# tkwong/parameter_server

Hardware: AMD Instinct MI355X
Metric: device-resident KV Add+Get GB/s (grad+param bytes) at 1/2/4/8 GPU (higher is better)
Workload: dtype f32; 1 GPU; cfg 2 dense: 1e8-key float shard, 64 x 1000000 contiguous-key windows at 1M-aligned bases pushed, then windows the push did not touch pulled (zero push/pull overlap), per step; assign (last-write-wins) mode, grouped launches, 16 window sets rotated over the steps; key_space=100000000, batch_keys=1000000, window_sets=16, push_pull_overlap_keys=0, parallelism=range-sharded x1 (no collective)

## Files before the change

### parameter_server_amd/csrc/pskv_internal.h

```cpp
#pragma once
#include <hip/hip_runtime.h>
#include <stddef.h>
#include <stdint.h>

#include "pskv_plan.h"

namespace pskv {

constexpr int kBlock = 256;
constexpr int kGatherVec = 4;
constexpr int kSortedUnroll = 2;
inline int stream_chunk(int unroll) { return kBlock * 4 * unroll; }
constexpr int kSortedChunk = kBlock * 4 * kSortedUnroll;
constexpr int kGeneralChunk = 2048;
constexpr int kGeneralSlots = 4096;
constexpr int kRbBinBlockDefault = 1024;
constexpr uint32_t kRbMaxSc = 1024;
constexpr int kInlineMax = 256;
constexpr int kInlineGetMax = 512;
constexpr int kInlineMaxChunks = 16;
constexpr unsigned long long kEmpty64 = ~0ull;
constexpr uint32_t kEmpty32 = 0xFFFFFFFFu;

constexpr uint32_t kErrOverflowFull = 1u;
// ... 77 lines not shown
};
static_assert(sizeof(OvfMbox) == 128, "device and host words on separate 64-byte lines");
struct OvfCtl {
  OvfTab t;
  uint32_t stat[2];
  OvfMbox* mbox;
};
struct Ovf {
  OvfCtl* c;
};

hipError_t launch_gather(int vb, bool vec, int unroll, bool nt, const GroupArgs& ga,
                         uint32_t nwg, const DenseView& d, const Ovf& o, hipStream_t st);
hipError_t launch_assign_sorted(int vb, bool vec, const uint32_t* keys, const void* vals,
                                uint64_t n, const DenseView& d, uint32_t* flag, uint32_t epoch,
                                hipStream_t st);
hipError_t launch_assign_group(int vb, bool vec, int unroll, bool nt, bool ntp, bool early,
                               const GroupArgs& ga,
                               const DenseView& d, uint32_t tile_shift, uint64_t ntiles,
                               uint32_t grid, uint32_t* flag, uint32_t epoch, hipStream_t st);
hipError_t launch_general_mark(int dtype, int mode, const GroupArgs& ga, uint32_t nwg,
                               const DenseView& d, uint32_t* oor, unsigned long long* owner,
                               const uint32_t* cond, uint32_t epoch, hipStream_t st);
hipError_t launch_general_commit(int vb, const GroupArgs& ga, uint32_t nwg, const DenseView& d,
                                 const unsigned long long* owner,
                                 const uint32_t* cond, uint32_t epoch, hipStream_t st);
hipError_t launch_ovf_rehash(int vb, const Ovf& o, uint64_t from_cap, const OvfTab& to, hipStream_t st);
hipError_t launch_replay(int dtype, int mode, const GroupArgs& ga, const DenseView& d, const Ovf& o,
                         const uint32_t* cond, uint32_t epoch, hipStream_t st, bool oor_only = false);
constexpr uint32_t kK1rTableWords = 4100;
hipError_t launch_gather_replay(int vb, bool vec, int unroll, bool nt, const GroupArgs& ga, uint32_t nwg,
                                const DenseView& d, const Ovf& o, const ReplayGroup& rg,
                                const uint32_t* cond, uint32_t epoch, uint32_t* tab, hipStream_t st);
hipError_t launch_rb_add(int dtype, int mode, const GroupArgs& ga, uint32_t nsc,
                         const DenseView& d, const Ovf& o, const RbMap& bm,
                         int apply_log2, int bin_block, uint16_t* loff, void* tmp,
                         hipStream_t st);
uint32_t rb_superchunk(int vb, int bin_block);
constexpr size_t kRbTmpPad = 16;
hipError_t launch_inline_add(int dtype, int mode, const InlineAdd& a, const DenseView& d,
                             const Ovf& o, hipStream_t st);
hipError_t launch_inline_get(int vb, const InlineGet& a, const DenseView& d, const Ovf& o,
                             void* out, unsigned int* done, unsigned int seq, hipStream_t st);
hipError_t launch_serve(int dtype, int mode, SrvRing* ring, const DenseView& d, const Ovf& o,
                        void* reply, uint32_t start_seq, unsigned long long idle_ticks,
                        uint32_t gen, hipStream_t st);
size_t rb_entry_bytes(int vb);
hipError_t launch_dense_check(const GroupArgs& ga, uint32_t nchunks, const DenseView& d,
                              uint32_t* flag, uint32_t epoch, hipStream_t st);
hipError_t launch_acc_dense(int dtype, const GroupArgs& ga, uint32_t grid, const DenseView& d,
                            const uint32_t* flag, uint32_t epoch, hipStream_t st);


struct RowShape {
  uint32_t units;
  uint32_t unit_bytes;
  uint32_t lanes;
  uint32_t lshift;
};
RowShape row_shape(uint32_t width, int vb, bool unit16);
hipError_t launch_row_gather(int vb, bool nt, const GroupArgs& ga, uint32_t nwg, const DenseView& d,
                             const RowShape& rs, hipStream_t st);
hipError_t launch_row_commit(int vb, const GroupArgs& ga, uint32_t nwg, const DenseView& d,
                             const unsigned long long* owner, const Ovf& o, uint32_t epoch,
                             const RowShape& rs, hipStream_t st);
hipError_t launch_row_accumulate(int dtype, const GroupArgs& ga, uint32_t nwg, const DenseView& d,
// ... 4 lines not shown
```

### parameter_server_amd/csrc/pskv_kernels.hip

```cpp
#include <type_traits>

#include "pskv_internal.h"

namespace pskv {
namespace {


__device__ __forceinline__ uint32_t fmix32(uint32_t h) {
  h ^= h >> 16;
  h *= 0x85ebca6bu;
  h ^= h >> 13;
  h *= 0xc2b2ae35u;
  h ^= h >> 16;
  return h;
}

typedef unsigned int u32x4 __attribute__((ext_vector_type(4)));

template <bool NT>
__device__ __forceinline__ u32x4 ld16(const void* p) {
  if (NT) return __builtin_nontemporal_load(reinterpret_cast<const u32x4*>(p));
  return *reinterpret_cast<const u32x4*>(p);
}
template <bool NT>
// ... 292 lines not shown
  if (run && (off0 & 3u) == 0u) {
    Vec4<VT>::template load<NTP>(reinterpret_cast<const VT*>(d.param) + off0, v);
  } else if (sizeof(VT) == 4 && run) {
    uint32_t t[4];
    ld16a4<NTP>(reinterpret_cast<const uint32_t*>(d.param) + off0, t);
#pragma unroll
    for (int e = 0; e < 4; ++e) v[e] = (VT)t[e];
  } else {
#pragma unroll
    for (int e = 0; e < 4; ++e) v[e] = load_one<VT, FRESH>(d, o, k[e]);
  }
}

template <bool FRESH = false>
__device__ __forceinline__ void gather2(const DenseView& d, const Ovf& o, const uint32_t (&k)[2],
                                        unsigned long long (&v)[2]) {
  using T = unsigned long long;
  const uint32_t off0 = k[0] - d.key_begin;
  const bool run = (k[1] == k[0] + 1u) & ((uint64_t)off0 + 1u < d.range);
  if (run && (off0 & 1u) == 0u) {
    Vec2x8::load(reinterpret_cast<const T*>(d.param) + off0, v);
  } else if (run) {
    uint32_t t[4];
    ld16a4<false>(reinterpret_cast<const uint32_t*>(reinterpret_cast<const T*>(d.param) + off0), t);
    v[0] = (T)t[0] | ((T)t[1] << 32);
    v[1] = (T)t[2] | ((T)t[3] << 32);
  } else {
    v[0] = load_one<T, FRESH>(d, o, k[0]);
    v[1] = load_one<T, FRESH>(d, o, k[1]);
  }
}

struct GoAlways {
  __device__ bool operator()() const { return true; }
};
template <typename VT, bool VEC, int U, bool NT, typename Go = GoAlways, bool FRESH = false>
__device__ __forceinline__ void gather_chunk(const GroupArgs& ga, const DenseView& d, const Ovf& o,
                                             uint32_t wg, Go go = Go()) {
  constexpr int CH = kBlock * 4 * U;
  const int j = batch_of(ga, wg);
  const uint32_t* __restrict__ keys = ga.b[j].keys;
  VT* __restrict__ out = reinterpret_cast<VT*>(const_cast<void*>(ga.b[j].vals));
  const uint64_t n = ga.b[j].n;
  const uint64_t base = (uint64_t)(wg - ga.wg_prefix[j]) * CH;
  const int tid = threadIdx.x;
  if constexpr (sizeof(VT) == 8) {
    if (VEC && base + CH <= n) {
      constexpr int UU = 2 * U;
      uint32_t k[UU][2];
#pragma unroll
      for (int u = 0; u < UU; ++u) ld8_keys<NT>(keys + base + (uint64_t)(u * kBlock + tid) * 2, k[u]);
      if (!go()) return;
      VT v[UU][2];
#pragma unroll
      for (int u = 0; u < UU; ++u) gather2<FRESH>(d, o, k[u], v[u]);
#pragma unroll
      for (int u = 0; u < UU; ++u) Vec2x8::store<NT>(out + base + (uint64_t)(u * kBlock + tid) * 2, v[u]);
      return;
    }
  }
  STEP_STAMP(1, 0);
  if (VEC && base + CH <= n) {
    uint32_t k[U][4];
#pragma unroll
    for (int u = 0; u < U; ++u)
      Vec4<uint32_t>::load<NT>(keys + base + (uint64_t)(u * kBlock + tid) * 4, k[u]);
    if (!go()) return;
#ifdef PSKV_STEP_STAMPS
    ready(k[0]);
    STEP_STAMP(1, 1);
#endif
    VT v[U][4];
#pragma unroll
    for (int u = 0; u < U; ++u) gather4<VT, false, FRESH>(d, o, k[u], v[u]);
#pragma unroll
    for (int u = 0; u < U; ++u)
      Vec4<VT>::template store<NT>(out + base + (uint64_t)(u * kBlock + tid) * 4, v[u]);
    STEP_STAMP(1, 2);
  } else {
    if (!go()) return;
    const uint64_t end = n < base + CH ? n : base + CH;
    for (uint64_t i0 = base + tid; i0 < end; i0 += 8ull * kBlock) {
      uint32_t kk[8];
      VT vv[8];
#pragma unroll
      for (int q = 0; q < 8; ++q) {
        const uint64_t i = i0 + (uint64_t)q * kBlock;
        kk[q] = i < end ? keys[i] : 0u;
      }
#pragma unroll
      for (int q = 0; q < 8; ++q)
        vv[q] = i0 + (uint64_t)q * kBlock < end ? load_one<VT, FRESH>(d, o, kk[q]) : VT(0);
#pragma unroll
      for (int q = 0; q < 8; ++q) {
        const uint64_t i = i0 + (uint64_t)q * kBlock;
        if (i < end) out[i] = vv[q];
      }
    }
  }
}

template <typename VT, bool VEC, int U, bool NT>
__global__ __launch_bounds__(kBlock) void k_gather(GroupArgs ga, DenseView d, Ovf o) {
  gather_chunk<VT, VEC, U, NT>(ga, d, o, blockIdx.x);
}


template <typename VT>
__device__ __forceinline__ bool scalar_elem(const uint32_t* __restrict__ keys,
                                            const VT* __restrict__ vals, uint64_t n, uint64_t i,
                                            const DenseView& d, uint64_t lo, uint64_t hi) {
  const uint32_t k = keys[i];
  const bool hn = i + 1 < n;
  const uint32_t nk = hn ? keys[i + 1] : 0u;
// ... 1368 lines not shown
          } else {
            const long long sl = ovf_insert(o, ot, key[q]);
            if (sl >= 0) reinterpret_cast<VT*>(ot.vals)[sl] = v[q];
          }
        } else {
          if (!(own >> q & 1u)) continue;
          VT* p = nullptr;
          if ((uint64_t)off < d.range) {
            p = reinterpret_cast<VT*>(d.param) + off;
          } else {
            const long long sl = ovf_insert(o, ot, key[q]);
            if (sl >= 0) p = reinterpret_cast<VT*>(ot.vals) + sl;
          }
          if (p) *p = add_wrap<VT>(*p, hsum[slot[q]]);
        }
      }
      __syncthreads();
    }
  }
}

template <typename VT, int MODE, bool OOR_ONLY>
__global__ __launch_bounds__(kReplayBlock) void k_replay(GroupArgs ga, DenseView d, Ovf o,
                                                         const uint32_t* cond, uint32_t epoch) {
  constexpr int SLOTS = replay_slots<kReplayBlock>();
  __shared__ uint32_t hk[SLOTS];
  __shared__ uint32_t hidx[MODE == 0 ? SLOTS + 1 : 1];
  __shared__ VT hsum[MODE == 1 ? SLOTS + 1 : 1];
  __shared__ uint32_t sent;
  if (*cond != epoch) return;
  replay_group<VT, MODE, kReplayBlock, GroupArgs, OOR_ONLY>(ga, d, o, hk, hidx, hsum, &sent);
}

template <typename VT, bool VEC, int U, bool NT>
__global__ __launch_bounds__(kBlock) void k_gather_r(GroupArgs ga, DenseView d, Ovf o, ReplayGroup rg,
                                                     const uint32_t* cond, uint32_t epoch, uint32_t* tab) {
  const uint32_t tag = *cond;
  bool tagged = false;
  gather_chunk<VT, VEC, U, NT>(ga, d, o, blockIdx.x, [&]() {
    tagged = tag == epoch;
    return !tagged;
  });
  if (tagged && blockIdx.x == 0) {
    constexpr int SLOTS = replay_slots<kBlock>();
    static_assert(2 * SLOTS + 2 <= (int)kK1rTableWords, "K1r's replay table fits its scratch");
    replay_group<VT, 0, kBlock>(rg, d, o, tab, tab + SLOTS, static_cast<VT*>(nullptr), tab + 2 * SLOTS + 1);
    for (uint32_t w = 0; w < gridDim.x; ++w) gather_chunk<VT, VEC, U, NT, GoAlways, true>(ga, d, o, w);
  }
}


template <int U>
__global__ __launch_bounds__(kBlock) void k_dense_check(GroupArgs ga, DenseView d, uint32_t* flag,
                                                        uint32_t epoch) {
  constexpr int CH = kBlock * 4 * U;
  const uint32_t wg = blockIdx.x;
  const int j = batch_of(ga, wg);
  const uint32_t* __restrict__ keys = ga.b[j].keys;
  const uint64_t n = ga.b[j].n;
  const uint64_t base = (uint64_t)(wg - ga.wg_prefix[j]) * CH;
  const int tid = threadIdx.x;
  const uint32_t first = keys[0];
  const uint64_t off = (uint32_t)(first - d.key_begin);
  bool bad = off >= d.range || off + n > d.range;
  if (base + CH <= n && (reinterpret_cast<uintptr_t>(keys) & 15u) == 0) {
    uint32_t k[U][4];
#pragma unroll
    for (int u = 0; u < U; ++u)
      Vec4<uint32_t>::load<true>(keys + base + (uint64_t)(u * kBlock + tid) * 4, k[u]);
#pragma unroll
    for (int u = 0; u < U; ++u) {
      const uint32_t k0 = first + (uint32_t)(base + (uint64_t)(u * kBlock + tid) * 4);
      bad |= (k[u][0] != k0) | (k[u][1] != k0 + 1u) | (k[u][2] != k0 + 2u) | (k[u][3] != k0 + 3u);
    }
  } else {
    const uint64_t end = n < base + CH ? n : base + CH;
    for (uint64_t i = base + tid; i < end; i += kBlock) bad |= keys[i] != first + (uint32_t)i;
  }
  if (__any(bad) && (tid & 63) == 0) *flag = epoch;
}
// ... 408 lines not shown
                                   const Ovf& o, const ReplayGroup& rg, const uint32_t* cond, uint32_t epoch,
                                   uint32_t* tab, hipStream_t st) {
  if (unroll == 8) {
    if (nt)
      k_gather_r<VT, VEC, 8, true><<<nwg, kBlock, 0, st>>>(ga, d, o, rg, cond, epoch, tab);
    else
      k_gather_r<VT, VEC, 8, false><<<nwg, kBlock, 0, st>>>(ga, d, o, rg, cond, epoch, tab);
  } else {
    if (nt)
      k_gather_r<VT, VEC, 4, true><<<nwg, kBlock, 0, st>>>(ga, d, o, rg, cond, epoch, tab);
    else
      k_gather_r<VT, VEC, 4, false><<<nwg, kBlock, 0, st>>>(ga, d, o, rg, cond, epoch, tab);
  }
}

hipError_t launch_gather_replay(int vb, bool vec, int unroll, bool nt, const GroupArgs& ga, uint32_t nwg,
                                const DenseView& d, const Ovf& o, const ReplayGroup& rg,
                                const uint32_t* cond, uint32_t epoch, uint32_t* tab, hipStream_t st) {
  if (nwg == 0) return hipErrorInvalidValue;
  if (vb == 4) {
    if (vec)
      gather_replay_dispatch<uint32_t, true>(unroll, nt, nwg, ga, d, o, rg, cond, epoch, tab, st);
    else
      gather_replay_dispatch<uint32_t, false>(unroll, nt, nwg, ga, d, o, rg, cond, epoch, tab, st);
  } else {
    if (vec)
      gather_replay_dispatch<unsigned long long, true>(unroll, nt, nwg, ga, d, o, rg, cond, epoch, tab, st);
    else
      gather_replay_dispatch<unsigned long long, false>(unroll, nt, nwg, ga, d, o, rg, cond, epoch, tab, st);
  }
  return hipGetLastError();
}

hipError_t launch_assign_sorted(int vb, bool vec, const uint32_t* keys, const void* vals,
                                uint64_t n, const DenseView& d, uint32_t* flag, uint32_t epoch,
                                hipStream_t st) {
  if (n == 0) return hipSuccess;
  const uint32_t nwg = (uint32_t)((n + kSortedChunk - 1) / kSortedChunk);
  if (vb == 4) {
    auto v = reinterpret_cast<const uint32_t*>(vals);
    if (vec)
      k_assign_sorted<uint32_t, true><<<nwg, kBlock, 0, st>>>(keys, v, n, d, flag, epoch);
    else
      k_assign_sorted<uint32_t, false><<<nwg, kBlock, 0, st>>>(keys, v, n, d, flag, epoch);
  } else {
    auto v = reinterpret_cast<const unsigned long long*>(vals);
    if (vec)
      k_assign_sorted<unsigned long long, true><<<nwg, kBlock, 0, st>>>(keys, v, n, d, flag, epoch);
    else
      k_assign_sorted<unsigned long long, false><<<nwg, kBlock, 0, st>>>(keys, v, n, d, flag, epoch);
  }
  return hipGetLastError();
}

#ifndef PSKV_K2G_LDS_CAP
#define PSKV_K2G_LDS_CAP (48u << 10)
#endif
constexpr uint32_t kK2gLdsCap = PSKV_K2G_LDS_CAP;

template <typename VT, bool VEC, bool NTP>
static void group_dispatch2(int unroll, bool nt, bool early, uint32_t grid, const GroupArgs& ga,
                            const DenseView& d, uint32_t shift, uint64_t ntiles, uint32_t* flag,
                            uint32_t epoch, hipStream_t st) {
  const uint32_t cap = sizeof(VT) == 4 && VEC && unroll == 8 ? kK2gLdsCap : 0u;
  if constexpr (sizeof(VT) == 4 && VEC) {
    if (early && unroll == 8 && nt) {
// ... 255 lines not shown
```

### parameter_server_amd/csrc/pskv_plan.h

```cpp
#pragma once
#include <stddef.h>
#include <stdint.h>

#include <algorithm>
#include <cstring>
#include <utility>
#include <vector>

#include "pskv.h"

namespace pskv {

constexpr int kMaxBatches = 64;
constexpr int kRbMaxBuckets = 2064;
constexpr uint64_t kMaxGroupElems = 1ull << 32;

constexpr size_t kPieceBytes = 1 << 20;
constexpr size_t kCheckPieceBytes = 256 << 10;
constexpr size_t kWindowBytes = 8 << 20;

namespace {

static inline size_t round16(size_t x) { return (x + 15) & ~size_t(15); }

// ... 17 lines not shown
                                             uint64_t max_elems = kMaxGroupElems) {
  std::vector<Span> out;
  size_t b = 0;
  while (b < v.size()) {
    size_t e = b;
    uint64_t el = 0;
    while (e < v.size() && e - b < max_batches && el + v[e].n < max_elems) {
      el += v[e].n;
      ++e;
    }
    out.emplace_back(b, e);
    b = e;
  }
  return out;
}

static inline std::vector<Span> batch_windows(const std::vector<pskv_batch>& v, size_t min_key_bytes = kWindowBytes,
                                              size_t max_batches = kMaxBatches,
                                              uint64_t max_elems = kMaxGroupElems) {
  std::vector<Span> wins;
  for (size_t i = 0; i < v.size();) {
    size_t j = i, kb = 0;
    uint64_t el = 0;
    while (j < v.size() &&
           (j == i || (kb < min_key_bytes && j - i < max_batches && el + v[j].n < max_elems))) {
      kb += v[j].n * 4;
      el += v[j].n;
      ++j;
    }
    wins.emplace_back(i, j);
    i = j;
  }
  return wins;
}

enum class StageOrder {
  kInterleaved,
  kKeysFirst,
};
struct StageSlot {
  size_t keys, vals;
};
struct StageLayout {
  std::vector<StageSlot> at;
  size_t key_bytes = 0;
  size_t total = 0;
  std::vector<pskv_batch> views(const std::vector<pskv_batch>& v, char* base) const {
    std::vector<pskv_batch> out(v.size());
    for (size_t i = 0; i < v.size(); ++i)
      out[i] = pskv_batch{reinterpret_cast<const uint32_t*>(base + at[i].keys), base + at[i].vals, v[i].n};
    return out;
  }
};

static inline size_t staged_bytes(const std::vector<pskv_batch>& v, size_t vb) {
  size_t bytes = 0;
  for (const auto& b : v) bytes += round16(b.n * 4) + round16(b.n * vb);
  return bytes;
}

static inline StageLayout stage_layout(const std::vector<pskv_batch>& v, size_t vb, StageOrder order) {
  StageLayout l;
  l.at.resize(v.size());
  for (const auto& b : v) l.key_bytes += round16(b.n * 4);
  size_t ko = 0, vo = order == StageOrder::kKeysFirst ? l.key_bytes : 0;
  for (size_t i = 0; i < v.size(); ++i) {
// ... 146 lines not shown
```

### parameter_server_amd/csrc/pskv_shard.cpp

```cpp
#include <hip/hip_runtime.h>

#include <algorithm>
#include <cctype>
#include <cerrno>
#include <atomic>
#include <chrono>
#include <condition_variable>
#include <cstdio>
#include <cstdlib>
#include <cstring>
#include <functional>
#include <mutex>
#include <string>
#include <thread>
#include <vector>

#include "pskv.h"
#include "pskv_frames.h"
#include "pskv_internal.h"
#include "pskv_plan.h"
#include "pskv_queues.h"

using namespace pskv;

// ... 197 lines not shown
  uint32_t tune_rb_wbits = 0;
  uint32_t tune_rb_nbd = 0;
  bool tune_inline = true;
  int tune_inline_add_chunks = 1;
  int tune_inline_get_chunks = 2;
  void* ireply = nullptr;
  bool tune_ispin = true;
  unsigned int ireply_seq = 0;
  int tune_rb_apply_log2 = 0;
  int tune_rb_bin_block = kRbBinBlockDefault;
  bool tune_serve = false;
  uint32_t tune_serve_idle_us = 20000;
  SrvRing* srv = nullptr;
  uint32_t srv_gen = 0;
  hipStream_t srv_stream = nullptr;
  hipEvent_t srv_dep = nullptr;
  bool srv_running = false;
  uint32_t srv_posted = 0;
  unsigned long long srv_idle_ticks = 0;
  bool counted = false;
  bool add_chunks_set = false;
  int wall_khz = 0;
  uint32_t tune_sync_timeout_ms = 120000;
  int last_kernel = -1;
  uint64_t launches = 0;
  hipEvent_t sync_ev = nullptr;
  uint32_t* stat_host = nullptr;
  int tune_fold_replay = 1;
  bool defer_replay = false;
  bool pend_replay = false;
  ReplayGroup pend_rg{};
  uint32_t pend_epoch = 0;
  uint64_t pend_elems = 0;

  DenseView dview() const { return DenseView{dense, key_begin, range}; }
};

namespace {

constexpr uint64_t kGetSmallKeys = 24ull << 20;
int gather_unroll(const pskv_shard* s, uint64_t elems) {
  if (s->tune_get_unroll) return s->tune_get_unroll;
  if (s->tune_unroll == 4) return 4;
  return elems < kGetSmallKeys ? 4 : 8;
}

int use_device(pskv_shard* s) {
  PSKV_HIP(hipSetDevice(s->device));
  return PSKV_OK;
}

hipEvent_t take_event(pskv_shard* s) {
  if (!s->event_pool.empty()) {
    hipEvent_t e = s->event_pool.back();
    s->event_pool.pop_back();
    return e;
  }
  hipEvent_t e = nullptr;
  if (hipEventCreateWithFlags(&e, hipEventDisableSystemFence) != hipSuccess) return nullptr;
  return e;
}

struct LaunchTimer {
  pskv_shard* s;
  int kernel;
  uint64_t elems;
// ... 1237 lines not shown
  if (s->width > 1) return rows_get(s, in, flags);
  std::vector<pskv_batch> v;
  for (auto& b : in) {
    if (b.n == 0) continue;
    if (!b.keys || !b.vals) return fail(PSKV_EINVAL, "pskv_get: null keys/out with n > 0");
    push_pieces(v, b, (size_t)s->vb);
  }
  s->n_get++;
  if (v.empty()) return PSKV_OK;
  int rc = use_device(s);
  if (rc) return rc;
  const bool device = (flags & PSKV_DEVICE) != 0;
  if (!device && s->tune_inline) {
    uint64_t total = 0;
    for (const auto& b : v) total += b.n;
    if (total <= (uint64_t)kInlineGetMax * s->tune_inline_get_chunks) return inline_get(s, v, total);
  }
  rc = srv_stop(s);
  if (rc) return rc;
  if (device) return gather_all(s, v, all_aligned16(v), true);
  const size_t bytes = staged_bytes(v, (size_t)s->vb);
  std::vector<pskv_batch> views;
  if (bytes <= s->tune_frame_zc_max_bytes &&
      (((flags & PSKV_HOST_FRAME) && frame_views(v, (size_t)s->vb, &views)) ||
       pinned_views(v, (size_t)s->vb, &views)))
    return zero_copy_get_views(s, views);
  bool pinned = true;
  for (const auto& b : v) pinned = pinned && is_pinned(b.keys) && is_pinned(b.vals);
  if (!pinned && s->tune_zc_max_bytes && bytes <= s->tune_zc_max_bytes) return zero_copy_get(s, v);
  if (!pinned && s->tune_pageable_dma) pinned = bytes >= s->tune_dma_min_bytes_get;
  return pinned ? pinned_get(s, v) : staged_get(s, v);
}

int add_get_impl(pskv_shard* s, const std::vector<pskv_batch>& adds, const std::vector<pskv_batch>& gets,
                 int flags) {
  if (s->width > 1) {
    const int rc = rows_add(s, adds, flags);
    return rc ? rc : rows_get(s, gets, flags);
  }
  s->defer_replay = s->tune_fold_replay && (flags & PSKV_DEVICE) && s->mode == PSKV_ASSIGN && s->vb == 4;
  int rc = add_impl(s, adds, flags);
  s->defer_replay = false;
  if (!rc) rc = get_impl(s, gets, flags & ~PSKV_SORTED_HINT);
  const int rf = flush_replay(s);
  return rc ? rc : rf;
}

struct Option {
  const char* name;
  int64_t lo, hi;
  int64_t (*get)(const pskv_shard*);
  void (*set)(pskv_shard*, int64_t);
};

#define PSKV_OPT(NAME, LO, HI, FIELD, T)                                           \
  Option {                                                                         \
    NAME, LO, HI, [](const pskv_shard* s) -> int64_t { return (int64_t)s->FIELD; }, \
        [](pskv_shard* s, int64_t v) { s->FIELD = (T)v; }                          \
  }

const Option kOptions[] = {
    PSKV_OPT("GENERAL", 0, 2, general_path, int),
    PSKV_OPT("UNROLL", 4, 8, tune_unroll, int),
    PSKV_OPT("GET_UNROLL", 0, 8, tune_get_unroll, int),
    PSKV_OPT("FOLD_REPLAY", 0, 1, tune_fold_replay, int),
    PSKV_OPT("NT", 0, 1, tune_nt, bool),
    PSKV_OPT("NTP", 0, 1, tune_ntp, bool),
    PSKV_OPT("EARLY", 0, 2, tune_early, int),
    PSKV_OPT("PAGEABLE_DMA", 0, 1, tune_pageable_dma, bool),
    PSKV_OPT("DMA_MIN_BYTES", 0, INT64_MAX, tune_dma_min_bytes, size_t),
    PSKV_OPT("DMA_MIN_BYTES_GET", 0, INT64_MAX, tune_dma_min_bytes_get, size_t),
    PSKV_OPT("DMA_MIN_BYTES_PINNED", 0, INT64_MAX, tune_dma_min_bytes_pinned, size_t),
    PSKV_OPT("ZC_MAX_BYTES", 0, INT64_MAX, tune_zc_max_bytes, size_t),
    PSKV_OPT("FRAME_ZC_MAX_BYTES", 0, INT64_MAX, tune_frame_zc_max_bytes, size_t),
    PSKV_OPT("INLINE", 0, 1, tune_inline, bool),
    PSKV_OPT("INLINE_ADD_CHUNKS", 1, kInlineMaxChunks, tune_inline_add_chunks, int),
    PSKV_OPT("INLINE_GET_CHUNKS", 1, kInlineMaxChunks, tune_inline_get_chunks, int),
    PSKV_OPT("ISPIN", 0, 1, tune_ispin, bool),
    PSKV_OPT("SERVE", 0, 1, tune_serve, bool),
    PSKV_OPT("SERVE_IDLE_US", 1, 10000000, tune_serve_idle_us, uint32_t),
    PSKV_OPT("TILE_SHIFT", 0, 20, tune_tile_shift, uint32_t),
    PSKV_OPT("TILE_GRID", 1, 65536, tune_tile_grid, uint32_t),
    PSKV_OPT("RB_WBITS", 0, 31, tune_rb_wbits, uint32_t),
    PSKV_OPT("RB_NBD", 0, kRbMaxBuckets - 1, tune_rb_nbd, uint32_t),
    PSKV_OPT("RB_TB", 0, 11, tune_rb_tb, uint32_t),
    PSKV_OPT("RB_APPLY_LOG2", 0, 14, tune_rb_apply_log2, int),
    PSKV_OPT("RB_BIN_BLOCK", 512, 1024, tune_rb_bin_block, int),
    PSKV_OPT("SYNC_TIMEOUT_MS", 0, 0x7FFFFFFF, tune_sync_timeout_ms, uint32_t),
};
#undef PSKV_OPT

const Option* find_option(const char* name) {
  for (const auto& o : kOptions)
    if (std::strcmp(o.name, name) == 0) return &o;
  return nullptr;
}

int set_option(pskv_shard* s, const Option& o, int64_t v) {
  if (v < o.lo || v > o.hi) return fail(PSKV_EINVAL, std::string("option ") + o.name + ": value out of range");
  if (std::strcmp(o.name, "UNROLL") == 0 && v != 4 && v != 8) return fail(PSKV_EINVAL, "option UNROLL: 4 or 8");
  if (std::strcmp(o.name, "GET_UNROLL") == 0 && v != 0 && v != 4 && v != 8)
    return fail(PSKV_EINVAL, "option GET_UNROLL: 0, 4 or 8");
  if (std::strcmp(o.name, "TILE_SHIFT") == 0 && v != 0 && v < 10) return fail(PSKV_EINVAL, "option TILE_SHIFT: 0 or 10..20");
  if (std::strcmp(o.name, "RB_APPLY_LOG2") == 0 && v != 0 && v != 13 && v != 14)
    return fail(PSKV_EINVAL, "option RB_APPLY_LOG2: 0, 13 or 14");
  if (std::strcmp(o.name, "RB_BIN_BLOCK") == 0 && v != 512 && v != 1024)
    return fail(PSKV_EINVAL, "option RB_BIN_BLOCK: 512 or 1024");
  o.set(s, v);
  if (std::strcmp(o.name, "SYNC_TIMEOUT_MS") == 0) refresh_grow_wait(s);
  if (std::strcmp(o.name, "INLINE_ADD_CHUNKS") == 0) s->add_chunks_set = true;
  if (std::strcmp(o.name, "SERVE") == 0 && !s->add_chunks_set) s->tune_inline_add_chunks = v ? 2 : 1;
  return PSKV_OK;
}

int apply_env_options(pskv_shard* s) {
  static std::mutex warn_mu;
  static std::vector<std::string> warned;
  static const char* const kRetired[] = {"RB_INSERT", "GET_DEDUP", "GET_NTP", "FUSE"};
  for (const char* name : kRetired) {
    const std::string var = std::string("PSKV_") + name;
    const char* e = std::getenv(var.c_str());
// ... 160 lines not shown
  if (s->out_stream) drain(s->out_stream, "D2H output stream (destroy)");
  if (s->own_stream) drain(s->own_stream, "shard stream (destroy)");
  if (s->stream && s->stream != s->own_stream) drain(s->stream, "caller stream (destroy)");
  if (!stuck.empty()) {
    std::fprintf(stderr, "pskv: shard destroy: %s; its device memory and streams are not freed\n", stuck.c_str());
    return fail(PSKV_ESTATE, "pskv_shard_destroy: " + stuck);
  }
  GrowService::get().remove(s);
  if (s->counted) g_queues.add_shard(s->device, -1);
  if (s->out_stream) g_queues.add_stream(s->device, -1);
  if (s->srv) (void)hipHostFree(s->srv);
  if (s->srv_stream) (void)hipStreamDestroy(s->srv_stream);
  if (s->srv_dep) (void)hipEventDestroy(s->srv_dep);
  if (s->out_stream) (void)hipStreamDestroy(s->out_stream);
  for (auto e : s->out_events) (void)hipEventDestroy(e);
  for (auto& t : s->pending) {
    (void)hipEventDestroy(t.a);
    (void)hipEventDestroy(t.b);
  }
  for (auto e : s->event_pool) (void)hipEventDestroy(e);
  if (s->sync_ev) (void)hipEventDestroy(s->sync_ev);
  if (s->dense) (void)hipFree(s->dense);
  if (s->owner) (void)hipFree(s->owner);
  if (s->flag) (void)hipFree(s->flag);
  for (const auto& t : s->tables) {
    (void)hipFree(t.keys);
    (void)hipFree(t.vals);
  }
  if (s->ovf.c) (void)hipFree(s->ovf.c);
  if (s->mbox) (void)hipHostFree(s->mbox);
  if (s->dstage) (void)hipFree(s->dstage);
  if (s->rb_loff) (void)hipFree(s->rb_loff);
  if (s->rb_ent) (void)hipFree(s->rb_ent);
  if (s->hstage) (void)hipHostFree(s->hstage);
  if (s->ireply) (void)hipHostFree(s->ireply);
  if (s->stat_host) (void)hipHostFree(s->stat_host);
  if (s->hstage_free) (void)hipEventDestroy(s->hstage_free);
  if (s->h2d_done) (void)hipEventDestroy(s->h2d_done);
  for (auto e : s->win_events) (void)hipEventDestroy(e);
  if (s->own_stream) (void)hipStreamDestroy(s->own_stream);
  delete s;
  return PSKV_OK;
}

static bool bad_flags(int flags) {
  return (flags & ~(PSKV_DEVICE | PSKV_SORTED_HINT | PSKV_HOST_FRAME)) != 0 ||
         ((flags & PSKV_DEVICE) && (flags & PSKV_HOST_FRAME));
}

int pskv_add(pskv_shard* s, const uint32_t* keys, const void* vals, uint64_t n, int flags) {
  if (!s) return fail(PSKV_EINVAL, "pskv_add: null shard");
  if (bad_flags(flags)) return fail(PSKV_EINVAL, "pskv_add: unknown flags");
  pskv_batch b{keys, const_cast<void*>(vals), n};
  return add_impl(s, std::vector<pskv_batch>{b}, flags);
}

int pskv_get(pskv_shard* s, const uint32_t* keys, uint64_t n, void* out, int flags) {
  if (!s) return fail(PSKV_EINVAL, "pskv_get: null shard");
  if (bad_flags(flags)) return fail(PSKV_EINVAL, "pskv_get: unknown flags");
  pskv_batch b{keys, out, n};
  return get_impl(s, std::vector<pskv_batch>{b}, flags);
}

int pskv_add_grouped(pskv_shard* s, const pskv_batch* batches, uint64_t nb, int flags) {
  if (!s) return fail(PSKV_EINVAL, "pskv_add_grouped: null shard");
  if (nb && !batches) return fail(PSKV_EINVAL, "pskv_add_grouped: null batches");
// ... 226 lines not shown
```

Measured before the change: 6432 GB/s.

## Fuse last push group and first pull group into one concurrent step kernel

Adds a fused step kernel that runs the final assign-add group's workgroups and the first gather group's workgroups in one launch. Gather workgroups check their key range against the push windows with wave ballots and defer any chunk that overlaps a push to a tail kernel, which also handles the replay fallback. A host-side rule reads a device-written report and stops fusing for a while when more than half of the chunks were deferred. The aim is to remove the serialization and launch gap between push and pull so read and write bandwidth overlap. The cost is extra overlap-check work, a tail launch, and added complexity.

New measurement: 6429 GB/s (median of 3 runs). No clear change (-0.0%).

```diff
diff --git a/parameter_server_amd/csrc/pskv_internal.h b/parameter_server_amd/csrc/pskv_internal.h
--- a/parameter_server_amd/csrc/pskv_internal.h
+++ b/parameter_server_amd/csrc/pskv_internal.h
@@ -133,6 +133,20 @@
 hipError_t launch_gather_replay(int vb, bool vec, int unroll, bool nt, const GroupArgs& ga, uint32_t nwg,
                                 const DenseView& d, const Ovf& o, const ReplayGroup& rg,
                                 const uint32_t* cond, uint32_t epoch, uint32_t* tab, hipStream_t st);
+struct FuseCtl {
+  uint32_t* defer;
+  uint32_t* total;
+  unsigned long long* report;
+};
+constexpr int kFuseUnroll = 4;
+static_assert(2 * sizeof(GroupArgs) + 160 <= 4096 && sizeof(GroupArgs) + sizeof(ReplayGroup) + 160 <= 4096,
+              "K10's and K1t's groups plus their other arguments fit the 4 KiB kernarg segment");
+hipError_t launch_step_fused(bool early, const GroupArgs& ga, uint32_t nadd, const GroupArgs& gg, uint32_t nget,
+                             const DenseView& d, const Ovf& o, uint32_t tile_shift, uint64_t ntiles,
+                             uint32_t* flag, uint32_t epoch, const FuseCtl& fc, hipStream_t st);
+hipError_t launch_gather_tail(const GroupArgs& gg, uint32_t nget, uint32_t grid, const DenseView& d, const Ovf& o,
+                              const ReplayGroup& rg, const uint32_t* cond, uint32_t epoch, uint32_t* tab,
+                              const FuseCtl& fc, hipStream_t st);
 hipError_t launch_rb_add(int dtype, int mode, const GroupArgs& ga, uint32_t nsc,
                          const DenseView& d, const Ovf& o, const RbMap& bm,
                          int apply_log2, int bin_block, uint16_t* loff, void* tmp,
diff --git a/parameter_server_amd/csrc/pskv_kernels.hip b/parameter_server_amd/csrc/pskv_kernels.hip
--- a/parameter_server_amd/csrc/pskv_kernels.hip
+++ b/parameter_server_amd/csrc/pskv_kernels.hip
@@ -348,7 +348,11 @@
 }
 
 struct GoAlways {
-  __device__ bool operator()() const { return true; }
+  template <typename K>
+  __device__ bool whole(const K&) const {
+    return true;
+  }
+  __device__ bool part(const uint32_t*, uint64_t, uint64_t) const { return true; }
 };
 template <typename VT, bool VEC, int U, bool NT, typename Go = GoAlways, bool FRESH = false>
 __device__ __forceinline__ void gather_chunk(const GroupArgs& ga, const DenseView& d, const Ovf& o,
@@ -366,7 +370,7 @@
       uint32_t k[UU][2];
 #pragma unroll
       for (int u = 0; u < UU; ++u) ld8_keys<NT>(keys + base + (uint64_t)(u * kBlock + tid) * 2, k[u]);
-      if (!go()) return;
+      if (!go.whole(k)) return;
       VT v[UU][2];
 #pragma unroll
       for (int u = 0; u < UU; ++u) gather2<FRESH>(d, o, k[u], v[u]);
@@ -381,7 +385,7 @@
 #pragma unroll
     for (int u = 0; u < U; ++u)
       Vec4<uint32_t>::load<NT>(keys + base + (uint64_t)(u * kBlock + tid) * 4, k[u]);
-    if (!go()) return;
+    if (!go.whole(k)) return;
 #ifdef PSKV_STEP_STAMPS
     ready(k[0]);
     STEP_STAMP(1, 1);
@@ -394,8 +398,8 @@
       Vec4<VT>::template store<NT>(out + base + (uint64_t)(u * kBlock + tid) * 4, v[u]);
     STEP_STAMP(1, 2);
   } else {
-    if (!go()) return;
     const uint64_t end = n < base + CH ? n : base + CH;
+    if (!go.part(keys, base, end)) return;
     for (uint64_t i0 = base + tid; i0 < end; i0 += 8ull * kBlock) {
       uint32_t kk[8];
       VT vv[8];
@@ -1830,20 +1834,230 @@
   replay_group<VT, MODE, kReplayBlock, GroupArgs, OOR_ONLY>(ga, d, o, hk, hidx, hsum, &sent);
 }
 
+struct GoUntagged {
+  uint32_t tag, epoch;
+  template <typename K>
+  __device__ bool whole(const K&) const {
+    return tag != epoch;
+  }
+  __device__ bool part(const uint32_t*, uint64_t, uint64_t) const { return tag != epoch; }
+};
 template <typename VT, bool VEC, int U, bool NT>
 __global__ __launch_bounds__(kBlock) void k_gather_r(GroupArgs ga, DenseView d, Ovf o, ReplayGroup rg,
                                                      const uint32_t* cond, uint32_t epoch, uint32_t* tab) {
   const uint32_t tag = *cond;
-  bool tagged = false;
-  gather_chunk<VT, VEC, U, NT>(ga, d, o, blockIdx.x, [&]() {
-    tagged = tag == epoch;
-    return !tagged;
-  });
-  if (tagged && blockIdx.x == 0) {
+  gather_chunk<VT, VEC, U, NT>(ga, d, o, blockIdx.x, GoUntagged{tag, epoch});
+  if (tag == epoch && blockIdx.x == 0) {
     constexpr int SLOTS = replay_slots<kBlock>();
     static_assert(2 * SLOTS + 2 <= (int)kK1rTableWords, "K1r's replay table fits its scratch");
     replay_group<VT, 0, kBlock>(rg, d, o, tab, tab + SLOTS, static_cast<VT*>(nullptr), tab + 2 * SLOTS + 1);
     for (uint32_t w = 0; w < gridDim.x; ++w) gather_chunk<VT, VEC, U, NT, GoAlways, true>(ga, d, o, w);
+  }
+}
+
+struct GoDisjoint {
+  const GroupArgs& push;
+  uint32_t epoch;
+  uint32_t* word;
+  uint32_t* total;
+  template <typename Hit>
+  __device__ __forceinline__ bool test(uint32_t lo, uint32_t hi, Hit hit) const {
+    const int lane = threadIdx.x & 63;
+    uint32_t pf = 0, pl = 0;
+    const bool pv = lane < push.nb && push.b[lane].n > 0;
+    if (pv) {
+      pf = push.b[lane].keys[0];
+      pl = push.b[lane].keys[push.b[lane].n - 1];
+    }
+#pragma unroll
+    for (int w = 32; w >= 1; w >>= 1) {
+      lo = min(lo, (uint32_t)__shfl_xor((int)lo, w, 64));
+      hi = max(hi, (uint32_t)__shfl_xor((int)hi, w, 64));
+    }
+    unsigned long long m = __ballot(pv && pf <= hi && pl >= lo);
+    bool h = false;
+    while (m) {
+      const int q = __ffsll((long long)m) - 1;
+      m &= m - 1;
+      h |= hit((uint32_t)__shfl((int)pf, q, 64), (uint32_t)__shfl((int)pl, q, 64));
+    }
+    if (__ballot(h) == 0) return true;
+    if (lane == 0 && atomicExch(word, epoch) != epoch) atomicAdd(total, 1u);
+    return false;
+  }
+  template <int UU>
+  __device__ __forceinline__ bool whole(const uint32_t (&k)[UU][4]) const {
+    uint32_t lo = k[0][0], hi = k[0][0];
+#pragma unroll
+    for (int u = 0; u < UU; ++u)
+#pragma unroll
+      for (int e = 0; e < 4; ++e) {
+        lo = min(lo, k[u][e]);
+        hi = max(hi, k[u][e]);
+      }
+    return test(lo, hi, [&](uint32_t f, uint32_t l) {
+      bool h = false;
+#pragma unroll
+      for (int u = 0; u < UU; ++u)
+#pragma unroll
+        for (int e = 0; e < 4; ++e) h |= (k[u][e] >= f) & (k[u][e] <= l);
+      return h;
+    });
+  }
+  __device__ __forceinline__ bool part(const uint32_t* __restrict__ keys, uint64_t base, uint64_t end) const {
+    uint32_t lo = kEmpty32, hi = 0u;
+    for (uint64_t i = base + threadIdx.x; i < end; i += kBlock) {
+      lo = min(lo, keys[i]);
+      hi = max(hi, keys[i]);
+    }
+    return test(lo, hi, [&](uint32_t f, uint32_t l) {
+      bool h = false;
+      for (uint64_t i = base + threadIdx.x; i < end; i += kBlock) h |= (keys[i] >= f) & (keys[i] <= l);
+      return h;
+    });
+  }
+};
+
+template <int U, bool EARLY>
+__device__ __forceinline__ void step_add_wg(const GroupArgs& ga, const DenseView& d, uint32_t tile_shift,
+                                            uint64_t ntiles, uint32_t* flag, uint32_t epoch, uint32_t wg,
+                                            uint32_t nwg) {
+  constexpr uint32_t CH = kBlock * 4 * U;
+  __shared__ uint64_t s_seg_s[kMaxBatches];
+  __shared__ uint64_t s_seg_e[kMaxBatches];
+  __shared__ uint32_t s_first[kMaxBatches];
+  __shared__ uint32_t s_last[kMaxBatches];
+  __shared__ unsigned long long s_mask;
+  __shared__ int s_dense;
+  const uint32_t tid = threadIdx.x;
+  const uint32_t lane = tid & 63u;
+  const bool mine = wg < ga.wg_prefix[ga.nb];
+  const int j = mine ? batch_of(ga, wg) : 0;
+  const uint32_t base = mine ? (wg - ga.wg_prefix[j]) * CH : 0u;
+  const uint32_t n = (uint32_t)ga.b[j].n;
+  const uint32_t end = !mine ? 0u : (n - base < CH ? n : base + CH);
+  const bool whole = end - base == CH;
+  const uint32_t* __restrict__ kc = ga.b[j].keys + base;
+  const uint32_t* __restrict__ vc = reinterpret_cast<const uint32_t*>(ga.b[j].vals) + base;
+  uint32_t k[U][4], v[U][4];
+  if (EARLY && whole) {
+#pragma unroll
+    for (int u = 0; u < U; ++u) {
+      const uint32_t o = ((uint32_t)u * kBlock + tid) * 4u;
+      Vec4<uint32_t>::load<true>(kc + o, k[u]);
+      Vec4<uint32_t>::load<true>(vc + o, v[u]);
+    }
+  }
+  const GroupEnds g = group_prologue(ga, d, flag, epoch, s_first, s_last, &s_dense);
+  __syncthreads();
+  bool bad = false;
+  if (!s_dense) {
+    bad = tile_mode<uint32_t, true>(ga, d, g, tile_shift, ntiles, wg, nwg, s_seg_s, s_seg_e, &s_mask);
+  } else if (mine) {
+    const uint32_t first = s_first[j];
+    const uint32_t c_lo = first + base, c_hi = first + (end - 1u);
+    const bool ov = (int)lane > j && (int)lane < ga.nb && s_first[lane] <= c_hi && s_last[lane] >= c_lo;
+    const unsigned long long later = __ballot(ov);
+    const bool covered = __ballot(ov && s_first[lane] <= c_lo && s_last[lane] >= c_hi) != 0;
+    uint32_t* __restrict__ pc = reinterpret_cast<uint32_t*>(d.param) + (first - d.key_begin) + base;
+    auto shadowed = [&](uint32_t key) {
+      unsigned long long m = later;
+      bool sh = false;
+      while (m) {
+        const int q = __ffsll((long long)m) - 1;
+        m &= m - 1;
+        sh |= (key >= s_first[q]) & (key <= s_last[q]);
+      }
+      return sh;
+    };
+    if (whole) {
+      if (!EARLY) {
+#pragma unroll
+        for (int u = 0; u < U; ++u) {
+          const uint32_t o = ((uint32_t)u * kBlock + tid) * 4u;
+          Vec4<uint32_t>::load<true>(kc + o, k[u]);
+          if (!covered) Vec4<uint32_t>::load<true>(vc + o, v[u]);
+        }
+      }
+#pragma unroll
+      for (int u = 0; u < U; ++u) {
+        const uint32_t o = ((uint32_t)u * kBlock + tid) * 4u;
+        const uint32_t k0 = c_lo + o;
+        const bool lbad = (k[u][0] != k0) | (k[u][1] != k0 + 1u) | (k[u][2] != k0 + 2u) | (k[u][3] != k0 + 3u);
+        bad |= lbad;
+        if (covered || lbad) continue;
+        if (later == 0) {
+          st16a4<true>(pc + o, v[u]);
+        } else {
+#pragma unroll
+          for (int e = 0; e < 4; ++e)
+            if (!shadowed(k0 + (uint32_t)e)) pc[o + e] = v[u][e];
+        }
+      }
+    } else {
+      const uint32_t len = end - base;
+      for (uint32_t i0 = tid; i0 < len; i0 += 4u * kBlock) {
+        uint32_t kk[4], vv[4];
+#pragma unroll
+        for (int q = 0; q < 4; ++q) {
+          const uint32_t i = i0 + (uint32_t)q * kBlock;
+          kk[q] = i < len ? kc[i] : c_lo + i;
+          vv[q] = i < len && !covered ? vc[i] : 0u;
+        }
+#pragma unroll
+        for (int q = 0; q < 4; ++q) {
+          const uint32_t i = i0 + (uint32_t)q * kBlock;
+          const bool ebad = kk[q] != c_lo + i;
+          bad |= ebad;
+          if (i < len && !covered && !ebad && !shadowed(c_lo + i)) pc[i] = vv[q];
+        }
+      }
+    }
+  }
+  if (bad) *flag = epoch;
+}
+
+template <int U, bool EARLY>
+__global__ __launch_bounds__(kBlock) __attribute__((amdgpu_waves_per_eu(8, 8))) void k_step_fused(GroupArgs ga, GroupArgs gg, DenseView d, Ovf o,
+                                                       uint32_t nadd, uint32_t tile_shift, uint64_t ntiles,
+                                                       uint32_t* flag, uint32_t epoch, FuseCtl fc) {
+  if (blockIdx.x >= nadd) {
+    const uint32_t c = blockIdx.x - nadd;
+    gather_chunk<uint32_t, true, U, true>(gg, d, o, c, GoDisjoint{ga, epoch, fc.defer + c, fc.total});
+    return;
+  }
+  step_add_wg<U, EARLY>(ga, d, tile_shift, ntiles, flag, epoch, blockIdx.x, nadd);
+}
+
+template <int U>
+__global__ __launch_bounds__(kBlock) void k_gather_tail(GroupArgs ga, DenseView d, Ovf o, ReplayGroup rg,
+                                                        const uint32_t* cond, uint32_t epoch, uint32_t* tab,
+                                                        FuseCtl fc, uint32_t nchunks) {
+  const uint32_t tag = *cond;
+  if (blockIdx.x == 0 && threadIdx.x == 0) {
+    const uint32_t t = agent_load(fc.total), p = fc.total[1];
+    fc.total[1] = t;
+    const unsigned long long e = (unsigned long long)epoch << 32;
+    __hip_atomic_store(fc.report, e | (uint32_t)(t - p), __ATOMIC_RELAXED, __HIP_MEMORY_SCOPE_SYSTEM);
+    __hip_atomic_store(fc.report + 1, e | nchunks, __ATOMIC_RELAXED, __HIP_MEMORY_SCOPE_SYSTEM);
+  }
+  if (tag == epoch) {
+    if (blockIdx.x != 0) return;
+    constexpr int SLOTS = replay_slots<kBlock>();
+    replay_group<uint32_t, 0, kBlock>(rg, d, o, tab, tab + SLOTS, static_cast<uint32_t*>(nullptr),
+                                      tab + 2 * SLOTS + 1);
+    for (uint32_t w = 0; w < nchunks; ++w) gather_chunk<uint32_t, true, U, true, GoAlways, true>(ga, d, o, w);
+    return;
+  }
+  const uint32_t lane = threadIdx.x & 63u;
+  for (uint64_t c0 = blockIdx.x; c0 < nchunks; c0 += 64ull * gridDim.x) {
+    const uint64_t c = c0 + (uint64_t)lane * gridDim.x;
+    unsigned long long m = __ballot(c < nchunks && agent_load(fc.defer + c) == epoch);
+    while (m) {
+      const int q = __ffsll((long long)m) - 1;
+      m &= m - 1;
+      gather_chunk<uint32_t, true, U, true>(ga, d, o, (uint32_t)(c0 + (uint64_t)q * gridDim.x));
+    }
   }
 }
 
@@ -2318,6 +2532,26 @@
   return hipGetLastError();
 }
 
+hipError_t launch_step_fused(bool early, const GroupArgs& ga, uint32_t nadd, const GroupArgs& gg, uint32_t nget,
+                             const DenseView& d, const Ovf& o, uint32_t tile_shift, uint64_t ntiles,
+                             uint32_t* flag, uint32_t epoch, const FuseCtl& fc, hipStream_t st) {
+  if (nadd == 0 || nget == 0) return hipErrorInvalidValue;
+  const uint32_t grid = nadd + nget;
+  if (early)
+    k_step_fused<kFuseUnroll, true><<<grid, kBlock, 0, st>>>(ga, gg, d, o, nadd, tile_shift, ntiles, flag, epoch, fc);
+  else
+    k_step_fused<kFuseUnroll, false><<<grid, kBlock, 0, st>>>(ga, gg, d, o, nadd, tile_shift, ntiles, flag, epoch, fc);
+  return hipGetLastError();
+}
+
+hipError_t launch_gather_tail(const GroupArgs& gg, uint32_t nget, uint32_t grid, const DenseView& d, const Ovf& o,
+                              const ReplayGroup& rg, const uint32_t* cond, uint32_t epoch, uint32_t* tab,
+                              const FuseCtl& fc, hipStream_t st) {
+  if (nget == 0 || grid == 0) return hipErrorInvalidValue;
+  k_gather_tail<kFuseUnroll><<<grid, kBlock, 0, st>>>(gg, d, o, rg, cond, epoch, tab, fc, nget);
+  return hipGetLastError();
+}
+
 hipError_t launch_assign_sorted(int vb, bool vec, const uint32_t* keys, const void* vals,
                                 uint64_t n, const DenseView& d, uint32_t* flag, uint32_t epoch,
                                 hipStream_t st) {
diff --git a/parameter_server_amd/csrc/pskv_plan.h b/parameter_server_amd/csrc/pskv_plan.h
--- a/parameter_server_amd/csrc/pskv_plan.h
+++ b/parameter_server_amd/csrc/pskv_plan.h
@@ -73,6 +73,28 @@
     i = j;
   }
   return wins;
+}
+
+constexpr uint64_t kFuseStepMaxKeys = 36ull << 20;
+constexpr uint32_t kFuseStepHold = 63;
+struct FuseStepRule {
+  uint32_t hold = 0;
+  uint32_t seen = 0;
+};
+static inline void fuse_step_report(FuseStepRule& r, uint32_t epoch, uint32_t deferred, uint32_t chunks) {
+  if (epoch == 0 || epoch == r.seen) return;
+  r.seen = epoch;
+  if (2ull * deferred > chunks) r.hold = kFuseStepHold;
+}
+static inline bool fuse_step_take(int opt, uint64_t keys, uint64_t max_keys, FuseStepRule& r) {
+  if (opt == 0) return false;
+  if (opt == 1) return true;
+  if (keys >= max_keys) return false;
+  if (r.hold) {
+    --r.hold;
+    return false;
+  }
+  return true;
 }
 
 enum class StageOrder {
diff --git a/parameter_server_amd/csrc/pskv_shard.cpp b/parameter_server_amd/csrc/pskv_shard.cpp
--- a/parameter_server_amd/csrc/pskv_shard.cpp
+++ b/parameter_server_amd/csrc/pskv_shard.cpp
@@ -253,6 +253,14 @@
   ReplayGroup pend_rg{};
   uint32_t pend_epoch = 0;
   uint64_t pend_elems = 0;
+  int tune_fuse_step = 2;
+  uint64_t tune_fuse_step_max_keys = kFuseStepMaxKeys;
+  uint32_t tune_fuse_tail_grid = 256;
+  FuseStepRule fuse_rule{};
+  uint32_t* fuse_defer = nullptr;
+  size_t fuse_defer_bytes = 0;
+  unsigned long long* fuse_report = nullptr;
+  uint64_t n_fused = 0;
 
   DenseView dview() const { return DenseView{dense, key_begin, range}; }
 };
@@ -1556,11 +1564,104 @@
   return pinned ? pinned_get(s, v) : staged_get(s, v);
 }
 
+int fused_step(pskv_shard* s, const std::vector<pskv_batch>& adds, const std::vector<pskv_batch>& gets, int flags,
+               bool* done) {
+  *done = false;
+  if (s->tune_fuse_step == 0 || s->mode != PSKV_ASSIGN || s->vb != 4 || !s->tune_nt || !s->tune_ntp) return PSKV_OK;
+  if (!s->tune_fold_replay) return PSKV_OK;
+  if ((flags & (PSKV_DEVICE | PSKV_SORTED_HINT)) != (PSKV_DEVICE | PSKV_SORTED_HINT)) return PSKV_OK;
+  uint64_t keys = 0, npush = 0, npull = 0;
+  for (const auto* in : {&adds, &gets})
+    for (const auto& b : *in) {
+      if (b.n == 0) continue;
+      if (!b.keys || !b.vals) return PSKV_OK;
+      if (!aligned16(b.keys) || !aligned16(b.vals)) return PSKV_OK;
+      keys += b.n;
+      ++(in == &adds ? npush : npull);
+    }
+  if (npush < 2 || npull == 0) return PSKV_OK;
+  if (s->fuse_report) {
+    const unsigned long long r0 = __atomic_load_n(&s->fuse_report[0], __ATOMIC_RELAXED),
+                             r1 = __atomic_load_n(&s->fuse_report[1], __ATOMIC_RELAXED);
+    if ((r0 >> 32) == (r1 >> 32)) fuse_step_report(s->fuse_rule, (uint32_t)(r0 >> 32), (uint32_t)r0, (uint32_t)r1);
+  }
+  if (!fuse_step_take(s->tune_fuse_step, keys, s->tune_fuse_step_max_keys, s->fuse_rule)) return PSKV_OK;
+  std::vector<pskv_batch> va, vg;
+  for (const auto& b : adds)
+    if (b.n) push_pieces(va, b, 4);
+  for (const auto& b : gets)
+    if (b.n) push_pieces(vg, b, 4);
+  const std::vector<Span> ag = split_groups(va), gg = split_groups(vg);
+  const Span al = ag.back(), gf = gg.front();
+  if (al.second - al.first < 2) return PSKV_OK;
+  const LaunchGroup A = make_group(va, al.first, al.second, stream_chunk(kFuseUnroll));
+  const LaunchGroup G = make_group(vg, gf.first, gf.second, stream_chunk(kFuseUnroll));
+  int rc = use_device(s);
+  if (rc) return rc;
+  if ((rc = srv_stop(s))) return rc;
+  if ((rc = flush_replay(s))) return rc;
+  if (!s->fuse_report) {
+    void* p = nullptr;
+    if (hipHostMalloc(&p, 2 * sizeof(unsigned long long), hipHostMallocCoherent) != hipSuccess)
+      return fail(PSKV_ENOMEM, "fused step report allocation failed");
+    s->fuse_report = static_cast<unsigned long long*>(p);
+    s->fuse_report[0] = s->fuse_report[1] = 0;
+  }
+  const size_t had = s->fuse_defer_bytes;
+  if ((rc = ensure_scratch(s, reinterpret_cast<void**>(&s->fuse_defer), &s->fuse_defer_bytes,
+                           (size_t)G.nwg * sizeof(uint32_t))))
+    return rc;
+  if (s->fuse_defer_bytes != had) PSKV_HIP(hipMemsetAsync(s->fuse_defer, 0, s->fuse_defer_bytes, s->stream));
+  *done = true;
+  s->n_add++;
+  s->n_get++;
+  for (size_t i = 0; i + 1 < ag.size(); ++i) {
+    if ((rc = sorted_add(s, va, ag[i].first, ag[i].second, true, next_epoch(s), true,
+                         true)))
+      return rc;
+  }
+  const uint32_t epoch = next_epoch(s);
+  uint32_t shift = 16;
+  while (shift > 12 && (A.elems >> shift) < 2048) --shift;
+  if (s->tune_tile_shift) shift = s->tune_tile_shift;
+  const uint64_t ntiles = (s->range + (1ull << shift) - 1) >> shift;
+  const uint32_t nadd =
+      (uint32_t)std::min<uint64_t>(std::max<uint64_t>(std::min<uint64_t>(ntiles, 1024), A.nwg), s->tune_tile_grid);
+  const bool early = s->tune_early == 1 || (s->tune_early == 2 && A.elems * 4 < s->range);
+  const FuseCtl fc{s->fuse_defer, s->flag + 2, s->fuse_report};
+  {
+    LaunchTimer t(s, PSKV_K_ASSIGN_TILES, A.elems);
+    PSKV_HIP(launch_step_fused(early, A.ga, nadd, G.ga, G.nwg, s->dview(), s->ovf, shift, ntiles, s->flag, epoch, fc,
+                               s->stream));
+    t.done();
+  }
+  s->n_sorted++;
+  s->n_fused++;
+  {
+    ReplayGroup rg;
+    rg.nb = A.ga.nb;
+    for (int i = 0; i < rg.nb; ++i) rg.b[i] = A.ga.b[i];
+    const uint32_t grid = s->tune_fuse_tail_grid ? std::min(G.nwg, s->tune_fuse_tail_grid) : G.nwg;
+    LaunchTimer t(s, PSKV_K_GATHER, G.elems);
+    PSKV_HIP(launch_gather_tail(G.ga, G.nwg, grid, s->dview(), s->ovf, rg, s->flag, epoch, s->flag + 16, fc,
+                                s->stream));
+    t.done();
+  }
+  for (size_t i = 1; i < gg.size(); ++i)
+    if ((rc = gather_group(s, vg, gg[i].first, gg[i].second, true, false))) return rc;
+  return PSKV_OK;
+}
+
 int add_get_impl(pskv_shard* s, const std::vector<pskv_batch>& adds, const std::vector<pskv_batch>& gets,
                  int flags) {
   if (s->width > 1) {
     const int rc = rows_add(s, adds, flags);
     return rc ? rc : rows_get(s, gets, flags);
+  }
+  {
+    bool done = false;
+    const int rc = fused_step(s, adds, gets, flags, &done);
+    if (rc || done) return rc;
   }
   s->defer_replay = s->tune_fold_replay && (flags & PSKV_DEVICE) && s->mode == PSKV_ASSIGN && s->vb == 4;
   int rc = add_impl(s, adds, flags);
@@ -1611,6 +1712,16 @@
     PSKV_OPT("RB_APPLY_LOG2", 0, 14, tune_rb_apply_log2, int),
     PSKV_OPT("RB_BIN_BLOCK", 512, 1024, tune_rb_bin_block, int),
     PSKV_OPT("SYNC_TIMEOUT_MS", 0, 0x7FFFFFFF, tune_sync_timeout_ms, uint32_t),
+    PSKV_OPT("FUSE_STEP", 0, 2, tune_fuse_step, int),
+    PSKV_OPT("FUSE_STEP_MAX_KEYS", 0, INT64_MAX, tune_fuse_step_max_keys, uint64_t),
+    PSKV_OPT("FUSE_TAIL_GRID", 0, 65536, tune_fuse_tail_grid, uint32_t),
+    Option{"FUSE_STEP_LAUNCHES", 0, -1, [](const pskv_shard* s) -> int64_t { return (int64_t)s->n_fused; },
+           [](pskv_shard*, int64_t) {}},
+    Option{"FUSE_STEP_DEFERRED", 0, -1,
+           [](const pskv_shard* s) -> int64_t {
+             return s->fuse_report ? (int64_t)(uint32_t)__atomic_load_n(&s->fuse_report[0], __ATOMIC_RELAXED) : 0;
+           },
+           [](pskv_shard*, int64_t) {}},
 };
 #undef PSKV_OPT
 
@@ -1837,6 +1948,8 @@
   if (s->dstage) (void)hipFree(s->dstage);
   if (s->rb_loff) (void)hipFree(s->rb_loff);
   if (s->rb_ent) (void)hipFree(s->rb_ent);
+  if (s->fuse_defer) (void)hipFree(s->fuse_defer);
+  if (s->fuse_report) (void)hipHostFree(s->fuse_report);
   if (s->hstage) (void)hipHostFree(s->hstage);
   if (s->ireply) (void)hipHostFree(s->ireply);
   if (s->stat_host) (void)hipHostFree(s->stat_host);
```
